# ipl-uw/ZeDO-Release

Hardware: AMD Instinct MI355X
Metric: poses/sec (1000-step sampler, H=50) (higher is better)
Workload: dtype f32; 1 GPU; BASELINE configs[2] (3DPW pw3d_test, H=50, 1000 steps): N=1015 poses/GPU x H=50 hypotheses, IPO 500 it (17 joints) + 1000 OIL steps + P1/P2 min-over-hypotheses selection; random-init ScoreModelFC_Adv weights, synthetic detections; settings=pw3d, rows_per_gpu=50750, poses_total=1015

## Files before the change

### include/zedo_hip.h

```cpp
#ifndef ZEDO_HIP_H
#define ZEDO_HIP_H

#include <stddef.h>
#include <stdint.h>

#ifdef __cplusplus
extern "C" {
#endif

#define ZEDO_ABI_VERSION 5

#define ZEDO_OK 0
#define ZEDO_E_BADARG (-1)
#define ZEDO_E_NOGPU (-2)
#define ZEDO_E_WORKSPACE (-3)

typedef struct zedo_weights zedo_weights_t;
typedef struct zedo_schedule zedo_schedule_t;

int zedo_abi_version(void);
const char *zedo_error_string(int code);

int zedo_weights_create(const float *h_params, size_t n_floats, int n_joints, int joint_dim, int hidden,
                        int embed, int n_blocks, void *stream, zedo_weights_t **out);
void zedo_weights_destroy(zedo_weights_t *w);

#define ZEDO_MATH_F32 0
#define ZEDO_MATH_F16X3 1
int zedo_weights_set_math(zedo_weights_t *w, int mode, void *stream);
int zedo_weights_get_math(const zedo_weights_t *w);

int zedo_schedule_create(const zedo_weights_t *w, const float *h_t, int S, float label_scale, float beta_min,
                         float beta_max, int n_sde, void *stream, zedo_schedule_t **out);
void zedo_schedule_destroy(zedo_schedule_t *s);
int zedo_schedule_read(const zedo_schedule_t *s, float *h_tbias, float *h_a, float *h_c);

size_t zedo_workspace_bytes(int B);

int zedo_reproj_prepare(const float *d_uv, const float *d_K, const float *d_conf, int N, int J,
                        float *d_geom, float *d_conf_clamped, void *stream);

int zedo_reproj_degenerate(const float *d_geom, int N, int J, int *h_count, void *stream);

// ... 47 lines not shown
```

### zedo-release_amd/csrc/zedo_capi.hip

```cpp
#include "../../include/zedo_hip.h"
#include "zedo_internal.h"

#include <algorithm>
#include <atomic>
#include <cmath>
#include <cstdlib>
#include <cstring>
#include <mutex>
#include <new>
#include <vector>

using namespace zedo;

struct zedo_weights {
    int J3, hidden, embed, n_blocks;
    float *d_all;
    const float *W_pre;
    const float *W_hid[4];
    const float *W_post;
    const float *b_post;
    const float *gamma[NLAYER], *beta[NLAYER];
    const float *W_s, *b_s;
    const float *W_t[NLAYER];
    const float *b_sum[NLAYER];
    float *d_scratch;
    std::mutex scratch_mu;
    int math;
    uint16_t *d_W16;
    float wmax_hid[6];
    float act_bound;
    float unscale[6];
    bool finite16;
    float row_ratio16;
};

struct zedo_schedule {
    int S, Sp, nl, hidden;
    float *d_tbias;
    std::vector<float> a, c;
};

#define HIPCHK(x)                      \
    do {                               \
        hipError_t e_ = (x);           \
        if (e_ != hipSuccess) return (int)e_; \
    } while (0)

static inline int round_up(int v, int m) { return (v + m - 1) / m * m; }
static int check_device();
static int check_device_fwd() { return check_device(); }

namespace {
struct Prof {
// ... 134 lines not shown
        case ZEDO_E_NOGPU: return "zedo: no gfx950 device";
        case ZEDO_E_WORKSPACE: return "zedo: workspace too small";
    }
    return code > 0 ? hipGetErrorString((hipError_t)code) : "zedo: unknown error";
}

static int check_device() {
    int dev = 0;
    if (hipGetDevice(&dev) != hipSuccess) return ZEDO_E_NOGPU;
    hipDeviceProp_t p;
    if (hipGetDeviceProperties(&p, dev) != hipSuccess) return ZEDO_E_NOGPU;
    if (strncmp(p.gcnArchName, "gfx950", 6) != 0) return ZEDO_E_NOGPU;
    return ZEDO_OK;
}

extern "C" int zedo_weights_create(const float *h_params, size_t n_floats, int n_joints, int joint_dim, int hidden,
                                   int embed, int n_blocks, void *stream, zedo_weights_t **out) {
    if (!h_params || !out) return ZEDO_E_BADARG;
    const int J3 = n_joints * joint_dim;
    if (hidden != HID || embed != EMB || n_blocks != 2 || J3 < 1 || J3 > XLD) return ZEDO_E_BADARG;
    const size_t H = hidden, E = embed;
    const size_t expect = (H * J3 + H) + (H * E + H) + 2 * H + (E * E + E) + 4 * ((H * H + H) + (H * E + H) + 2 * H) +
                          ((size_t)J3 * H + J3);
    if (n_floats != expect) return ZEDO_E_BADARG;
    if (int rc = check_device()) return rc;
    hipStream_t st = (hipStream_t)stream;

    size_t off = 0;
    auto take = [&](size_t n) { size_t o = off; off += (n + 63) / 64 * 64; return o; };
    const size_t o_Wpre = take(H * XLD), o_Whid0 = take(4 * H * H), o_Wpost = take((size_t)XLD * H), o_bpost = take(XLD);
    const size_t o_gamma = take(NLAYER * H), o_beta = take(NLAYER * H), o_Ws = take(E * E), o_bs = take(E);
    const size_t o_Wt = take(NLAYER * H * E), o_bsum = take(NLAYER * H);
    std::vector<float> img(off, 0.0f);

    const float *p = h_params;
    auto next = [&](size_t n) { const float *q = p; p += n; return q; };
    float wmax_hid_tmp[6] = {0, 0, 0, 0, 0, 0};
    float gn_bound[NLAYER] = {0, 0, 0, 0, 0};
    bool finite = true;
    auto all_finite = [&](const float *v, size_t n) {
        for (size_t q = 0; q < n; ++q) finite &= (bool)std::isfinite(v[q]);
    };
    float row_ratio = 1.0f;
    auto row_ratio_of = [&](const float *wm, size_t rows, size_t cols, float mat_max) {
        if (!(mat_max > 0.f)) return;
        for (size_t r = 0; r < rows; ++r) {
            float rm = 0.f;
// ... 29 lines not shown
        for (size_t q = 0; q < H * H; ++q) wm = std::fmax(wm, std::fabs(w[q]));
        all_finite(w, H * H);
        wmax_hid_tmp[l - 1] = wm;
        row_ratio_of(w, H, H, wm);
        memcpy(&img[o_Wt + (size_t)l * H * E], wt, sizeof(float) * H * E);
        memcpy(&img[o_gamma + (size_t)l * H], g, sizeof(float) * H);
        memcpy(&img[o_beta + (size_t)l * H], be, sizeof(float) * H);
        for (size_t n = 0; n < H; ++n) img[o_bsum + (size_t)l * H + n] = bt[n] + b[n];
    }
    const float *w_post = next((size_t)J3 * H), *b_post = next(J3);
    memcpy(&img[o_Wpost], w_post, sizeof(float) * J3 * H);
    for (size_t q = 0; q < (size_t)J3 * H; ++q) wmax_hid_tmp[5] = std::fmax(wmax_hid_tmp[5], std::fabs(w_post[q]));
    all_finite(w_post, (size_t)J3 * H);
    row_ratio_of(w_post, J3, H, wmax_hid_tmp[5]);
    memcpy(&img[o_bpost], b_post, sizeof(float) * J3);

    zedo_weights *w = new (std::nothrow) zedo_weights();
    if (!w) return (int)hipErrorOutOfMemory;
    w->J3 = J3; w->hidden = hidden; w->embed = embed; w->n_blocks = n_blocks;
    w->d_scratch = nullptr;
    w->math = ZEDO_MATH_F32; w->d_W16 = nullptr;
    for (int l = 0; l < 6; ++l) { w->wmax_hid[l] = wmax_hid_tmp[l]; w->unscale[l] = 1.0f; }
    w->act_bound = std::fmax(std::fmax(gn_bound[1], gn_bound[3]), gn_bound[0] + gn_bound[2] + gn_bound[4]);
    w->finite16 = finite;
    w->row_ratio16 = row_ratio;
    hipError_t e = hipMalloc(&w->d_all, off * sizeof(float));
    if (e == hipSuccess) e = hipMalloc(&w->d_scratch, sizeof(float) * ((size_t)2 * ROW_PAD * EMB + ROW_PAD));
    if (e != hipSuccess) { (void)hipFree(w->d_all); delete w; return (int)e; }
    e = hipMemcpyAsync(w->d_all, img.data(), off * sizeof(float), hipMemcpyHostToDevice, st);
    if (e == hipSuccess) e = hipStreamSynchronize(st);
    if (e != hipSuccess) { (void)hipFree(w->d_all); (void)hipFree(w->d_scratch); delete w; return (int)e; }
    const float *d = w->d_all;
    w->W_pre = d + o_Wpre;
    for (int l = 0; l < 4; ++l) w->W_hid[l] = d + o_Whid0 + (size_t)l * H * H;
    w->W_post = d + o_Wpost; w->b_post = d + o_bpost;
    for (int l = 0; l < NLAYER; ++l) {
        w->gamma[l] = d + o_gamma + (size_t)l * H; w->beta[l] = d + o_beta + (size_t)l * H;
        w->W_t[l] = d + o_Wt + (size_t)l * H * E;  w->b_sum[l] = d + o_bsum + (size_t)l * H;
    }
    w->W_s = d + o_Ws; w->b_s = d + o_bs;
    *out = w;
    return ZEDO_OK;
}

extern "C" void zedo_weights_destroy(zedo_weights_t *w) {
    if (!w) return;
    (void)hipFree(w->d_all);
    (void)hipFree(w->d_scratch);
    (void)hipFree(w->d_W16);
    delete w;
}

extern "C" int zedo_weights_get_math(const zedo_weights_t *w) { return w ? w->math : ZEDO_E_BADARG; }

extern "C" int zedo_weights_set_math(zedo_weights_t *w, int mode, void *stream) {
// ... 37 lines not shown
    s->a.resize(S); s->c.resize(S);
    for (int i = 0; i < S; ++i) {
        const double t = (double)h_t[i] * ((double)label_scale / 999.0), b0 = (double)beta_min, b1 = (double)beta_max;
        const double beta = b0 + t * (b1 - b0);
        const double disc = 1.0 - std::exp(-2.0 * b0 * t - (b1 - b0) * t * t);
        const double sd = 1.0 - std::exp(2.0 * (-0.25 * t * t * (b1 - b0) - 0.5 * t * b0));
        s->a[i] = (float)(1.0 + 0.5 * beta / n_sde);
        s->c[i] = (float)(-(beta * disc) / (n_sde * sd));
#ifdef ZEDO_MUT_SDE_C
        s->c[i] = (float)(-(beta * disc) / (n_sde * sd) * (1.0 + 1e-4));
#endif
    }
    const bool borrow = Sp == ROW_PAD;
    std::unique_lock<std::mutex> lk(const_cast<zedo_weights_t *>(w)->scratch_mu, std::defer_lock);
    float *d_t = nullptr, *d_pe = nullptr, *d_temb = nullptr;
    s->d_tbias = nullptr;
    hipError_t e = hipSuccess;
    if (borrow) {
        lk.lock();
        d_pe = w->d_scratch; d_temb = d_pe + (size_t)ROW_PAD * EMB; d_t = d_temb + (size_t)ROW_PAD * EMB;
    } else {
        e = hipMalloc(&d_t, sizeof(float) * S);
        if (e == hipSuccess) e = hipMalloc(&d_pe, sizeof(float) * (size_t)Sp * EMB);
        if (e == hipSuccess) e = hipMalloc(&d_temb, sizeof(float) * (size_t)Sp * EMB);
    }
    if (e == hipSuccess) e = hipMalloc(&s->d_tbias, sizeof(float) * (size_t)Sp * NLAYER * HID);
    if (e == hipSuccess) e = hipMemcpyAsync(d_t, h_t, sizeof(float) * S, hipMemcpyHostToDevice, st);
    if (e == hipSuccess) e = launch_posemb(d_t, S, Sp, label_scale, d_pe, st);
    if (e == hipSuccess) {
        LayerArgs a{};
        a.X = d_pe; a.ldx = EMB; a.W = w->W_s; a.ldw = EMB; a.bias = w->b_s; a.out = d_temb; a.ldo = EMB;
        a.K = EMB; a.N = EMB; a.Mp = Sp;
        e = launch_layer(a, EPI_BIAS_SILU, st);
    }
    for (int l = 0; l < NLAYER && e == hipSuccess; ++l) {
        LayerArgs a{};
        a.X = d_temb; a.ldx = EMB; a.W = w->W_t[l]; a.ldw = EMB; a.bias = w->b_sum[l];
        a.out = s->d_tbias + (size_t)l * HID; a.ldo = NLAYER * HID; a.K = EMB; a.N = HID; a.Mp = Sp;
        e = launch_layer(a, EPI_BIAS, st);
    }
    {
        const hipError_t es = hipStreamSynchronize(st);
        if (e == hipSuccess) e = es;
    }
    if (!borrow) { (void)hipFree(d_t); (void)hipFree(d_pe); (void)hipFree(d_temb); }
    if (e != hipSuccess) { (void)hipFree(s->d_tbias); delete s; return (int)e; }
    *out = s;
    return ZEDO_OK;
}

extern "C" void zedo_schedule_destroy(zedo_schedule_t *s) {
    if (!s) return;
    (void)hipFree(s->d_tbias);
    delete s;
}

extern "C" int zedo_schedule_read(const zedo_schedule_t *s, float *h_tbias, float *h_a, float *h_c) {
    if (!s) return ZEDO_E_BADARG;
    if (h_tbias) HIPCHK(hipMemcpy(h_tbias, s->d_tbias, sizeof(float) * (size_t)s->S * NLAYER * HID, hipMemcpyDeviceToHost));
    if (h_a) memcpy(h_a, s->a.data(), sizeof(float) * s->S);
    if (h_c) memcpy(h_c, s->c.data(), sizeof(float) * s->S);
    return ZEDO_OK;
}

static inline size_t ws_rows(int B) { return (size_t)round_up((int)std::min((size_t)B, chunk_rows_cap()), BATCH_PAD); }

extern "C" size_t zedo_workspace_bytes(int B) {
    if (B < 1) return 0;
// ... 33 lines not shown
    int solve = 0, B = 0, N = 0;
    long long row0 = 0;
};

struct Net {
    const zedo_weights *w;
    float *xpad, *h, *h1;
    int Bp, ld;
    hipStream_t st;
    bool f16() const { return w->math == ZEDO_MATH_F16X3; }
    const uint16_t *W_pre16() const { return w->d_W16 + 4 * (size_t)HID * HID * 2; }
    const uint16_t *W_post16() const { return W_pre16() + (size_t)HID * XLD * 2; }

    LayerArgs pre_args(const float *tb) const {
        LayerArgs a{};
        a.Mp = Bp; a.X = xpad; a.ldx = XLD; a.W = w->W_pre; a.ldw = XLD; a.K = XLD; a.N = HID;
        a.kzero8 = w->J3 <= XLD - 8;
        a.bias = tb; a.gamma = w->gamma[0]; a.beta = w->beta[0]; a.out = h; a.ldo = HID;
        return a;
    }
    Layer16Args pre_args16(const float *tb) const {
        Layer16Args b{};
        b.K = XLD; b.N = HID; b.Mp = Bp; b.ldo = ld; b.Xf32 = xpad; b.W = W_pre16(); b.unscale = w->unscale[4];
        b.bias = tb; b.gamma = w->gamma[0]; b.beta = w->beta[0]; b.out = h; b.out_f32 = 0;
        return b;
    }
    LayerArgs post_args(bool sde, float sa, float sc, float *eps_out, const NextReproj &nr) const {
        LayerArgs a{};
        a.Mp = Bp; a.X = h; a.ldx = HID; a.W = w->W_post; a.ldw = HID; a.K = HID; a.N = XLD; a.bias = w->b_post; a.ldo = XLD;
        a.scratch = h1 + (size_t)Bp * XLD;
        if (sde) {
            a.out = xpad; a.sde_a = sa; a.sde_c = sc;
            a.rp_geom = nr.geom; a.rp_T = nr.T; a.rp_solve = nr.solve; a.rp_B = nr.B; a.rp_N = nr.N; a.rp_row0 = nr.row0;
// ... 26 lines not shown
            const int l1 = 1 + 2 * blk, l2 = 2 + 2 * blk;
            if (f16()) {
                const size_t per = (size_t)HID * HID * 2;
                Layer16Args b{};
                b.K = HID; b.N = HID; b.Mp = Bp; b.ldx = b.ldo = ld; b.out_f32 = 0;
                b.X = reinterpret_cast<const uint16_t *>(h); b.W = w->d_W16 + (size_t)(l1 - 1) * per; b.unscale = w->unscale[l1 - 1];
                b.bias = tb + (size_t)l1 * HID; b.gamma = w->gamma[l1]; b.beta = w->beta[l1]; b.out = h1;
                { ProfScope ps(ZEDO_PROF_HIDDEN, st); b.clk = ps.clk; e = launch_layer16(b, EPI_GN_SILU, st); b.clk = nullptr; }
                if (e != hipSuccess) break;
                b.X = reinterpret_cast<const uint16_t *>(h1); b.W = w->d_W16 + (size_t)(l2 - 1) * per; b.unscale = w->unscale[l2 - 1];
                b.bias = tb + (size_t)l2 * HID; b.gamma = w->gamma[l2]; b.beta = w->beta[l2];
                b.res = reinterpret_cast<const uint16_t *>(h); b.out = h;
                { ProfScope ps(ZEDO_PROF_HIDDEN, st); b.clk = ps.clk; e = launch_layer16(b, EPI_GN_SILU_RES, st); b.clk = nullptr; }
            } else {
                LayerArgs a{};
                a.Mp = Bp; a.X = h; a.ldx = HID; a.W = w->W_hid[l1 - 1]; a.ldw = HID; a.K = HID; a.N = HID;
                a.bias = tb + (size_t)l1 * HID; a.gamma = w->gamma[l1]; a.beta = w->beta[l1]; a.out = h1; a.ldo = HID;
                { ProfScope ps(ZEDO_PROF_HIDDEN, st); a.clk = ps.clk; e = launch_layer(a, EPI_GN_SILU, st); a.clk = nullptr; }
                if (e != hipSuccess) break;
                a.X = h1; a.W = w->W_hid[l2 - 1];
                a.bias = tb + (size_t)l2 * HID; a.gamma = w->gamma[l2]; a.beta = w->beta[l2]; a.out = h;
                { ProfScope ps(ZEDO_PROF_HIDDEN, st); a.clk = ps.clk; e = launch_layer(a, EPI_GN_SILU_RES, st); a.clk = nullptr; }
            }
        }
        return e;
    }
    hipError_t post(bool sde, float sa, float sc, float *eps_out, const NextReproj &nr) const {
        ProfScope ps(ZEDO_PROF_POST, st);
        if (f16()) return launch_layer16(post_args16(sde, sa, sc, eps_out, nr), sde ? EPI_SDE : EPI_BIAS, st);
        return launch_layer(post_args(sde, sa, sc, eps_out, nr), sde ? EPI_SDE : EPI_BIAS, st);
    }
    hipError_t all(const float *tb, bool sde, float sa, float sc, float *eps_out, const NextReproj &nr = NextReproj()) const {
        hipError_t e = pre(tb);
        if (e == hipSuccess) e = hidden(tb);
        if (e == hipSuccess) e = post(sde, sa, sc, eps_out, nr);
        return e;
    }
};

struct Ws { float *xpad, *h, *h1; size_t rows; };
static Ws carve(void *ws, int B) {
    Ws r; r.rows = ws_rows(B);
    r.xpad = (float *)ws; r.h = r.xpad + r.rows * XLD; r.h1 = r.h + r.rows * HID;
    return r;
}

static int step_common(const zedo_weights_t *w, const zedo_schedule_t *s, int step, const float *d_x_in, float *d_out,
                       bool sde, int B, void *ws, size_t ws_bytes, hipStream_t st) {
    if (!w || !s || !d_x_in || !d_out || !ws || B < 1 || step < 0 || step >= s->S) return ZEDO_E_BADARG;
    if (ws_bytes < zedo_workspace_bytes(B)) return ZEDO_E_WORKSPACE;
    const size_t cap = chunk_rows_cap();
    const float *tb = s->d_tbias + (size_t)step * NLAYER * HID;
    for (size_t r0 = 0; r0 < (size_t)B; r0 += cap) {
        const int Bc = (int)std::min(cap, (size_t)B - r0), Bp = round_up(Bc, BATCH_PAD);
        Ws k = carve(ws, B);
        HIPCHK(launch_pack_rows(d_x_in + r0 * w->J3, k.xpad, Bc, Bp, w->J3, st));
        const Net net{w, k.xpad, k.h, k.h1, Bp, (int)k.rows, st};
        if (sde) {
            HIPCHK(net.all(tb, true, s->a[step], s->c[step], nullptr));
            HIPCHK(launch_unpack_rows(k.xpad, d_out + r0 * w->J3, Bc, w->J3, st));
        } else {
            HIPCHK(net.all(tb, false, 0.f, 0.f, k.h1));
            HIPCHK(launch_unpack_rows(k.h1, d_out + r0 * w->J3, Bc, w->J3, st));
        }
    }
    return ZEDO_OK;
}
// ... 24 lines not shown
        Ws k = carve(d_workspace, B);
        HIPCHK(launch_pack_rows(d_x + r0 * w->J3, k.xpad, Bc, Bp, w->J3, st));
        static const bool unfused = getenv("ZEDO_UNFUSED_REPROJ") != nullptr;
        const Net net{w, k.xpad, k.h, k.h1, Bp, (int)k.rows, st};
        for (int i = step_begin; i < step_end; ++i) {
            if (i == step_begin || unfused) {
                ProfScope ps(ZEDO_PROF_REPROJ, st);
                HIPCHK(launch_reproj_step_padded(k.xpad, d_geom, d_T + r0 * 3, i >= switch_step, Bc, N,
                                                 row_offset + (long long)r0, st));
            }
            NextReproj nr;
            if (i + 1 < step_end && !unfused) {
                nr.geom = d_geom; nr.T = d_T + r0 * 3; nr.solve = (i + 1) >= switch_step; nr.B = Bc; nr.N = N;
                nr.row0 = row_offset + (long long)r0;
            }
            HIPCHK(net.all(s->d_tbias + (size_t)i * NLAYER * HID, true, s->a[i], s->c[i], nullptr, nr));
        }
        HIPCHK(launch_unpack_rows(k.xpad, d_x + r0 * w->J3, Bc, w->J3, st));
    }
    return ZEDO_OK;
}

extern "C" int zedo_ipo_fit_resume(const float *d_x0, const float *d_uv, const float *d_K, const int *h_keylist, int k,
                                   int axes_mask, float ipo_T, float min_scale, float max_scale, int iters,
                                   double normaliser, float *d_R, float *d_T, float *d_q, float *d_scale,
                                   float *d_state, int it_begin, int B, int H, int N, int J, long long row_offset,
                                   void *stream) {
    if (!d_x0 || !d_uv || !d_K || !h_keylist || !d_R || !d_T || B < 1 || H < 1 || N < 1 || J < 1 || k < 1 || k > 17 ||
        iters < 0 || it_begin < 0 || (it_begin > 0 && !d_state) || !(normaliser > 0) || row_offset < 0)
        return ZEDO_E_BADARG;
    if (row_offset + (long long)B > (long long)H * N) return ZEDO_E_BADARG;
// ... 38 lines not shown
```

### zedo-release_amd/csrc/zedo_gemm.hip

```cpp
#include "zedo_internal.h"
#include "zedo_tile.h"

#include <atomic>
#include <cstdlib>

#ifdef ZEDO_UBENCH
#include "../../tools/ubench/zedo_tile_hooks.inc"
#else
#define TL_MARK(var)
#define TL_FLUSH(t0, t1, t2)
#endif

namespace zedo {

template <int BM, int BN, int WM, int WN, int EPI, int NBUF = 2, int BK = 32, int SCHED = 0, int KSKIP = 0, int KQ = 1>
__device__ __forceinline__ void layer_tile(const LayerArgs &a, const int m0, const int n0, const int out_m0) {
    constexpr int NW = WM * WN;
    constexpr int CPR = BK / 4;
    constexpr int RPD = 64 / CPR;
    constexpr int KG = BK / 8;
    static_assert(BK == 32 || BK == 16, "BK");
    constexpr int TM = BM / WM, TN = BN / WN;
    constexpr int TJ = TM / 32, TI = TN / 32;
    constexpr int IA = BN / RPD / NW, IB = BM / RPD / NW;
// ... 27 lines not shown
        else
            dma16(Xbase + (size_t)kt * (BK * 4) + (size_t)(p - IA) * (RPD * 4) * a.ldx, xlane,
                  lds0 + (unsigned)(((NBUF * BN + buf * BM + (wid * IB + (p - IA)) * RPD) * BK) * 4));
    };
    auto dma = [&](int kt, int buf) {
#pragma unroll
        for (int p = 0; p < IPW; ++p) dma_one(kt, buf, p);
    };

    const int fswz = (BK == 32) ? (li & 7) : ((li >> 2) & 3);
    int foff[KG];
#pragma unroll
    for (int kg = 0; kg < KG; ++kg) foff[kg] = ((2 * kg + kh) ^ fswz) * 4;
    const float *Ab0 = As + (wn * TN + li) * BK;
    const float *Bb0 = Bs + (wm * TM + li) * BK;
    f32x4 fa0[TI], fb0[TJ], fa1[TI], fb1[TJ];
    auto fread = [&](f32x4(&fa)[TI], f32x4(&fb)[TJ], int buf, int kg) {
#pragma unroll
        for (int i = 0; i < TI; ++i) fa[i] = *reinterpret_cast<const f32x4 *>(Ab0 + (buf * BN + i * 32) * BK + foff[kg]);
#pragma unroll
        for (int j = 0; j < TJ; ++j) fb[j] = *reinterpret_cast<const f32x4 *>(Bb0 + (buf * BM + j * 32) * BK + foff[kg]);
    };
    f32x16 acc[TI][TJ];
#pragma unroll
    for (int i = 0; i < TI; ++i)
#pragma unroll
        for (int j = 0; j < TJ; ++j)
#pragma unroll
            for (int e = 0; e < 16; ++e) acc[i][j][e] = 0.0f;
    auto mma = [&](const f32x4(&fa)[TI], const f32x4(&fb)[TJ]) {
#pragma unroll
        for (int e = 0; e < 4; ++e)
#pragma unroll
            for (int i = 0; i < TI; ++i)
#pragma unroll
                for (int j = 0; j < TJ; ++j)
                    acc[i][j] = __builtin_amdgcn_mfma_f32_32x32x2f32(fa[i][e], fb[j][e], acc[i][j], 0, 0, 0);
    };
    constexpr int H1 = (IPW + 1) / 2, H2 = IPW - H1;
    auto mma_dma = [&](const f32x4(&fa)[TI], const f32x4(&fb)[TJ], int kt, int buf, int p0, int cnt) {
#pragma unroll
        for (int e = 0; e < 4; ++e) {
#pragma unroll
            for (int q = 0; q < 4; ++q)
                if (q < cnt && q * 4 / cnt == e) {
                    dma_one(kt, buf, p0 + q);
                    __builtin_amdgcn_sched_barrier(0);
// ... 12 lines not shown
    TL_MARK(tl0)
    if (EPI != EPI_PARTIAL && tid < BN / 4) {
        *reinterpret_cast<f32x4 *>(Ps + tid * 4) = *reinterpret_cast<const f32x4 *>(a.bias + n0 + tid * 4);
        if constexpr (EPI == EPI_GN_SILU || EPI == EPI_GN_SILU_RES) {
            *reinterpret_cast<f32x4 *>(Ps + BN + tid * 4) = *reinterpret_cast<const f32x4 *>(a.gamma + n0 + tid * 4);
            *reinterpret_cast<f32x4 *>(Ps + 2 * BN + tid * 4) = *reinterpret_cast<const f32x4 *>(a.beta + n0 + tid * 4);
        }
    }
    const int KT = a.K / BK;
    f32x16 qsum[KQ > 1 ? TI : 1][KQ > 1 ? TJ : 1];
    const int KTQ = KT / KQ;
#pragma unroll
    for (int t = 0; t < NBUF; ++t) dma(min(t, KT - 1), t);
    asm volatile("s_waitcnt vmcnt(%0)" ::"n"((NBUF - 1) * IPW) : "memory");
    __syncthreads();
    fread(fa0, fb0, 0, 0);
    TL_MARK(tl1)
    for (int kt0 = 0; kt0 < KT; kt0 += NBUF) {
#pragma unroll
      for (int buf = 0; buf < NBUF; ++buf) {
        const int kt = kt0 + buf;
        const int nxt = (buf + 1 == NBUF) ? 0 : buf + 1;
        const int prv = (buf == 0) ? NBUF - 1 : buf - 1;
        fread(fa1, fb1, buf, 1);
        if constexpr (SCHED & 1) __builtin_amdgcn_sched_barrier(0);
        if constexpr (SCHED & 2) mma_dma(fa0, fb0, min(kt - 1 + NBUF, KT - 1), prv, H1, H2);
        else mma(fa0, fb0);
        if constexpr (KG == 4) {
            fread(fa0, fb0, buf, 2);
            if constexpr (SCHED & 1) __builtin_amdgcn_sched_barrier(0);
            mma(fa1, fb1);
            if constexpr (SCHED & 1) __builtin_amdgcn_sched_barrier(0);
            fread(fa1, fb1, buf, 3);
            if constexpr (SCHED & 1) __builtin_amdgcn_sched_barrier(0);
            mma(fa0, fb0);
        }
        const bool skip_last = KSKIP == 1 && KG == 4 && buf == NBUF - 1;
        asm volatile("s_waitcnt vmcnt(%0)" ::"n"((NBUF - 2) * IPW) : "memory");
        __syncthreads();
        if (skip_last) {
        } else if constexpr (SCHED & 2) {
            fread(fa0, fb0, nxt, 0);
            __builtin_amdgcn_sched_barrier(0);
            mma_dma(fa1, fb1, min(kt + NBUF, KT - 1), buf, 0, H1);
        } else {
            dma(min(kt + NBUF, KT - 1), buf);
            fread(fa0, fb0, nxt, 0);
            if constexpr (SCHED & 1) __builtin_amdgcn_sched_barrier(0);
            mma(fa1, fb1);
            if constexpr (SCHED & 1) __builtin_amdgcn_sched_barrier(0);
        }
      }
// ... 44 lines not shown
                    __builtin_amdgcn_global_load_lds(
                        (const __attribute__((address_space(1))) void *)(reinterpret_cast<const char *>(obase) +
                                                                         ((unsigned)grow * (unsigned)a.ldo + (unsigned)((pos ^ (sr & 7)) * 4)) * 4u),
                        (__attribute__((address_space(3))) void *)(S + idx * RPI * BN), 16, 0, 0);
                }
                asm volatile("s_waitcnt vmcnt(0)" ::: "memory");
                __syncthreads();
            }
#pragma unroll
            for (int i = 0; i < TI; ++i) {
                float o[16];
                f32x4 b4[4], ga[4], be[4];
                const float *pc = Ps + wn * TN + i * 32 + 4 * kh;
#pragma unroll
                for (int g = 0; g < 4; ++g) {
                    b4[g] = *reinterpret_cast<const f32x4 *>(pc + 8 * g);
                    if constexpr (EPI == EPI_GN_SILU || EPI == EPI_GN_SILU_RES) {
                        ga[g] = *reinterpret_cast<const f32x4 *>(pc + BN + 8 * g);
                        be[g] = *reinterpret_cast<const f32x4 *>(pc + 2 * BN + 8 * g);
                    }
                }
                epilogue_values<EPI>(acc[i][j], b4, ga, be, a.sde_c, o);
                float *srow = S + (wm * 32 + li) * BN;
#pragma unroll
                for (int g = 0; g < 4; ++g) {
                    const int c = (wn * TN + i * 32 + 8 * g + 4 * kh) >> 2;
                    f32x4 *slot = reinterpret_cast<f32x4 *>(srow + ((c ^ (li & 7)) << 2));
                    f32x4 v = {o[4 * g], o[4 * g + 1], o[4 * g + 2], o[4 * g + 3]};
                    if constexpr (EPI == EPI_GN_SILU_RES) {
                        const f32x4 h = *slot;
#pragma unroll
                        for (int e = 0; e < 4; ++e) v[e] += h[e];
                    } else if constexpr (EPI == EPI_SDE) {
                        const f32x4 x = *slot;
#pragma unroll
                        for (int e = 0; e < 4; ++e) v[e] = __builtin_fmaf(a.sde_a, x[e], v[e]);
                    }
// ... 133 lines not shown
        if (a.Mp % bm) return 1e30;
        const long tiles = (long)(a.Mp / bm) * ncol;
        const long rounds = (tiles + (long)cus * slots_per_cu - 1) / ((long)cus * slots_per_cu);
        return rounds * 6.0 + (double)((tiles + cus - 1) / cus) * tile_us;
    };
    const double kdepth = a.K / 1024.0;
    const double c32 = cost(32, 3, 14.5 * kdepth), c64 = cost(64, 3, 28.2 * kdepth), c128 = cost(128, 2, 55.1 * kdepth);
    if (c32 <= c64 && c32 <= c128) return launch_cfg<32, 128, 1, 4, EPI, 2, 32, SCHED_THIN>(a, st);
    if (c64 <= c128) return launch_cfg<64, 128, 2, 4, EPI, 2, 32, SCHED_THIN>(a, st);
    return launch_cfg<128, 128, 2, 2, EPI, 2, 32, SCHED_BIG, PLAIN_WPE>(a, st);
}

template <int EPI>
static hipError_t launch_wide(const LayerArgs &a, hipStream_t st) {
    if (a.K <= 64) {
        if (a.K == 64 && a.kzero8) return launch_cfg<64, 128, 2, 4, EPI, 2, 32, SCHED_THIN, 1, 1>(a, st);
        return launch_cfg<64, 128, 2, 4, EPI, 2, 32, SCHED_THIN>(a, st);
    }
    constexpr int WG_PER_CU = 3;
    constexpr int W8 = (EPI == EPI_GN_SILU_RES) ? 1 : 0;
    const int per_round = num_cus() * WG_PER_CU * 128 / (a.N / 128);
    int rows_big = (a.Mp / per_round) * per_round;
    if (rows_big == 0) {
        const int one_each = num_cus() * 128 / (a.N / 128);
        const int mix_big = (a.Mp / one_each) * one_each;
        constexpr int SMR = (W8 ? 64 : 32);
        if (mix_big > 0 && a.Mp > mix_big && (a.Mp - mix_big) % SMR == 0) {
            const double kd = a.K / 1024.0;
            const long small_tiles = (long)((a.Mp - mix_big) / SMR) * (a.N / 128);
            const double est_mix = (mix_big / one_each) * 55.1 * kd + (double)((small_tiles + num_cus() - 1) / num_cus()) * (W8 ? 28.2 : 13.9) * kd + 6.0;
            auto single = [&](int bm, int slots, double t) {
// ... 137 lines not shown
```

### zedo-release_amd/csrc/zedo_internal.h

```cpp
#pragma once
#include <hip/hip_runtime.h>
#include <stddef.h>
#include <stdint.h>

#include <atomic>

namespace zedo {

constexpr int MAX_DEVICES = 16;
inline int device_slot() {
    int dev = 0;
    if (hipGetDevice(&dev) != hipSuccess) return -1;
    return (dev >= 0 && dev < MAX_DEVICES) ? dev : -1;
}
inline hipError_t allow_lds(const void *kern, size_t lds, std::atomic<bool> *done ) {
    const int slot = device_slot();
    if (slot < 0 || !done[slot].load(std::memory_order_acquire)) {
        hipError_t e = hipFuncSetAttribute(kern, hipFuncAttributeMaxDynamicSharedMemorySize, (int)lds);
        if (e != hipSuccess) return e;
        if (slot >= 0) done[slot].store(true, std::memory_order_release);
    }
    return hipSuccess;
}
inline int num_cus() {
// ... 26 lines not shown
    EPI_PARTIAL = 5,
};

struct LayerArgs {
    const float *X;
    const float *W;
    const float *bias;
    const float *gamma;
    const float *beta;
    float *out;
    int ldx, ldw, ldo;
    int K;
    int N;
    int Mp;
    float sde_a, sde_c;
    int kzero8;
    long long *clk;
    const float *rp_geom;
    float *rp_T;
    int rp_solve, rp_B, rp_N;
    long long rp_row0;
    float *scratch;
};
constexpr int POST_SPLIT_ROWS = 2048;

hipError_t launch_layer(const LayerArgs &a, int epilogue, hipStream_t st);

struct Layer16Args {
    const uint16_t *X;
    int ldx, ldo;
    const uint16_t *W;
// ... 88 lines not shown
```

### zedo-release_amd/csrc/zedo_tile.h

```cpp
#pragma once
#include "zedo_internal.h"

namespace zedo {

typedef float f32x16 __attribute__((ext_vector_type(16)));
typedef float f32x2 __attribute__((ext_vector_type(2)));
typedef _Float16 f16x8 __attribute__((ext_vector_type(8)));
typedef _Float16 f16x4 __attribute__((ext_vector_type(4)));

__device__ __forceinline__ void split_f16x8(const f32x4 &v0, const f32x4 &v1, f16x8 &h, f16x8 &l) {
#pragma unroll
    for (int e = 0; e < 4; ++e) {
        const _Float16 h0 = (_Float16)v0[e], h1 = (_Float16)v1[e];
        h[e] = h0; h[4 + e] = h1;
        l[e] = (_Float16)(v0[e] - (float)h0); l[4 + e] = (_Float16)(v1[e] - (float)h1);
    }
}
__device__ __forceinline__ float join_f16(_Float16 h, _Float16 l) { return (float)h + (float)l; }


__device__ __forceinline__ void dma16(const char *sbase, unsigned voff, unsigned lds_byte_addr) {
    unsigned keep;
    asm volatile("s_mov_b32 %0, m0\n\ts_mov_b32 m0, %3\n\ts_nop 0\n\tglobal_load_lds_dwordx4 %2, %1\n\ts_mov_b32 m0, %0"
                 : "=&s"(keep)
// ... 3 lines not shown

template <int N>
__device__ __forceinline__ void dma16n(const char *sbase, unsigned voff, unsigned lds_byte_addr) {
    static_assert(N == 1 || N == 2 || N == 4, "pieces per M0 write (offsets up to 3072 fit the 13-bit signed field)");
    unsigned keep;
    if constexpr (N == 4)
        asm volatile("s_mov_b32 %0, m0\n\ts_mov_b32 m0, %3\n\ts_nop 0\n\tglobal_load_lds_dwordx4 %2, %1\n\tglobal_load_lds_dwordx4 %2, %1 offset:1024\n\t"
                     "global_load_lds_dwordx4 %2, %1 offset:2048\n\tglobal_load_lds_dwordx4 %2, %1 offset:3072\n\ts_mov_b32 m0, %0"
                     : "=&s"(keep) : "s"(sbase), "v"(voff), "s"(lds_byte_addr) : "memory");
    else if constexpr (N == 2)
        asm volatile("s_mov_b32 %0, m0\n\ts_mov_b32 m0, %3\n\ts_nop 0\n\tglobal_load_lds_dwordx4 %2, %1\n\tglobal_load_lds_dwordx4 %2, %1 offset:1024\n\ts_mov_b32 m0, %0"
                     : "=&s"(keep) : "s"(sbase), "v"(voff), "s"(lds_byte_addr) : "memory");
    else
        asm volatile("s_mov_b32 %0, m0\n\ts_mov_b32 m0, %3\n\ts_nop 0\n\tglobal_load_lds_dwordx4 %2, %1\n\ts_mov_b32 m0, %0"
                     : "=&s"(keep) : "s"(sbase), "v"(voff), "s"(lds_byte_addr) : "memory");
}

__device__ __forceinline__ float silu_fast(float y) {
    return y * __builtin_amdgcn_rcpf(1.0f + __builtin_amdgcn_exp2f(y * -1.44269504088896340736f));
}

template <int EPI, bool SCALED = false, bool PACKED = true>
__device__ __forceinline__ void epilogue_values(const f32x16 &acc, const f32x4 (&b4)[4], const f32x4 (&ga)[4],
                                                const f32x4 (&be)[4], float sde_c, float (&o)[16], float acc_scale = 1.0f) {
    if constexpr ((EPI == EPI_GN_SILU || EPI == EPI_GN_SILU_RES) && !PACKED) {
        float p[16];
#pragma unroll
        for (int k = 0; k < 16; ++k) {
            const float b = b4[k >> 2][k & 3];
            if constexpr (SCALED) p[k] = __builtin_fmaf(acc[k], acc_scale, b);
// ... 97 lines not shown
```

### zedo-release_amd/zedo_hip/__init__.py

```python
import ctypes
import os

import numpy as np
import torch

_HERE = os.path.dirname(os.path.abspath(__file__))


def _load_zedo_build():
    import importlib.util
    import sys
    if "zedo_build" in sys.modules:
        return sys.modules["zedo_build"]
    spec = importlib.util.spec_from_file_location("zedo_build", os.path.join(os.path.dirname(_HERE), "zedo_build.py"))
    mod = importlib.util.module_from_spec(spec)
    sys.modules["zedo_build"] = mod
    spec.loader.exec_module(mod)
    return mod


_zb = _load_zedo_build()

LIB_PATH = _zb.ensure_library()

_lib = ctypes.CDLL(LIB_PATH)

_vp, _i, _f, _d, _ll, _sz = (ctypes.c_void_p, ctypes.c_int, ctypes.c_float, ctypes.c_double,
                             ctypes.c_longlong, ctypes.c_size_t)

SIGNATURES = {
    "zedo_abi_version": (_i, []),
    "zedo_error_string": (ctypes.c_char_p, [_i]),
    "zedo_weights_create": (_i, [_vp, _sz, _i, _i, _i, _i, _i, _vp, ctypes.POINTER(_vp)]),
    "zedo_weights_destroy": (None, [_vp]),
    "zedo_weights_set_math": (_i, [_vp, _i, _vp]),
    "zedo_weights_get_math": (_i, [_vp]),
    "zedo_schedule_create": (_i, [_vp, _vp, _i, _f, _f, _f, _i, _vp, ctypes.POINTER(_vp)]),
    "zedo_schedule_destroy": (None, [_vp]),
    "zedo_schedule_read": (_i, [_vp, _vp, _vp, _vp]),
    "zedo_workspace_bytes": (_sz, [_i]),
    "zedo_reproj_prepare": (_i, [_vp, _vp, _vp, _i, _i, _vp, _vp, _vp]),
    "zedo_reproj_degenerate": (_i, [_vp, _i, _i, _vp, _vp]),
    "zedo_reproj_grad": (_i, [_vp, _vp, _vp, _i, _vp, _i, _i, _i, _ll, _vp]),
    "zedo_score_eps": (_i, [_vp, _vp, _i, _vp, _vp, _i, _vp, _sz, _vp]),
    "zedo_sde_step": (_i, [_vp, _vp, _i, _vp, _i, _vp, _sz, _vp]),
    "zedo_oil_run": (_i, [_vp, _vp, _vp, _vp, _vp, _i, _i, _i, _i, _i, _ll, _vp, _sz, _vp]),
    "zedo_ipo_fit": (_i, [_vp, _vp, _vp, _vp, _i, _i, _f, _f, _f, _i, _d, _vp, _vp, _vp, _vp, _i, _i, _i, _i, _ll, _vp]),
    "zedo_ipo_fit_resume": (_i, [_vp, _vp, _vp, _vp, _i, _i, _f, _f, _f, _i, _d, _vp, _vp, _vp, _vp, _vp, _i, _i, _i, _i,
                                 _i, _ll, _vp]),
    "zedo_rotate_init": (_i, [_vp, _vp, _vp, _i, _i, _i, _i, _ll, _vp]),
    "zedo_min_mpjpe": (_i, [_vp, _vp, _i, _i, _i, _ll, _i, _vp, _vp, _vp, _vp]),
# ... 342 lines not shown
```

Baseline: 319.3 poses/s.

## Fold GroupNorm mean-centring into pre-centred weights and biases for f32 path

Precomputes, at weight load, copies of the pre, hidden and time-embedding weights and biases with the GroupNorm per-group (32-channel) mean subtracted. The GEMM output is then already centred, so the epilogue only needs a variance reduction. The biases are loaded into the accumulators at init instead of being added afterwards. The gamma and beta are pre-scaled by -log2(e) so the SiLU exp2 needs fewer ops. It also adds a K-skip variant that drops more zero-padded K slices in the first layer. This costs extra weight and tbias memory, and changes the rounding of the f32 path.

Measured after the change: 320.9 poses/s, median of 6. About the same (+0.5%).

```diff
diff --git a/include/zedo_hip.h b/include/zedo_hip.h
--- a/include/zedo_hip.h
+++ b/include/zedo_hip.h
@@ -27,6 +27,7 @@
 
 #define ZEDO_MATH_F32 0
 #define ZEDO_MATH_F16X3 1
+int zedo_gn_centre(const float *h_in, int rows, int cols, float *h_out);
 int zedo_weights_set_math(zedo_weights_t *w, int mode, void *stream);
 int zedo_weights_get_math(const zedo_weights_t *w);
 
diff --git a/zedo-release_amd/csrc/zedo_capi.hip b/zedo-release_amd/csrc/zedo_capi.hip
--- a/zedo-release_amd/csrc/zedo_capi.hip
+++ b/zedo-release_amd/csrc/zedo_capi.hip
@@ -23,6 +23,8 @@
     const float *W_s, *b_s;
     const float *W_t[NLAYER];
     const float *b_sum[NLAYER];
+    const float *W_pre_c, *W_hid_c[4], *W_t_c[NLAYER], *b_sum_c[NLAYER];
+    const float *gamma_f[NLAYER], *beta_f[NLAYER];
     float *d_scratch;
     std::mutex scratch_mu;
     int math;
@@ -37,6 +39,7 @@
 struct zedo_schedule {
     int S, Sp, nl, hidden;
     float *d_tbias;
+    float *d_tbias_c;
     std::vector<float> a, c;
 };
 
@@ -201,6 +204,23 @@
     return ZEDO_OK;
 }
 
+static void gn_centre(const float *in, size_t rows, size_t cols, float *out) {
+    std::vector<double> m(cols);
+    for (size_t g = 0; g < rows; g += 32) {
+        std::fill(m.begin(), m.end(), 0.0);
+        for (size_t r = g; r < g + 32; ++r)
+            for (size_t c = 0; c < cols; ++c) m[c] += (double)in[r * cols + c];
+        for (size_t r = g; r < g + 32; ++r)
+            for (size_t c = 0; c < cols; ++c) out[r * cols + c] = (float)((double)in[r * cols + c] - m[c] * (1.0 / 32.0));
+    }
+}
+
+extern "C" int zedo_gn_centre(const float *h_in, int rows, int cols, float *h_out) {
+    if (!h_in || !h_out || rows < 32 || rows % 32 || cols < 1) return ZEDO_E_BADARG;
+    gn_centre(h_in, (size_t)rows, (size_t)cols, h_out);
+    return ZEDO_OK;
+}
+
 extern "C" int zedo_weights_create(const float *h_params, size_t n_floats, int n_joints, int joint_dim, int hidden,
                                    int embed, int n_blocks, void *stream, zedo_weights_t **out) {
     if (!h_params || !out) return ZEDO_E_BADARG;
@@ -218,6 +238,8 @@
     const size_t o_Wpre = take(H * XLD), o_Whid0 = take(4 * H * H), o_Wpost = take((size_t)XLD * H), o_bpost = take(XLD);
     const size_t o_gamma = take(NLAYER * H), o_beta = take(NLAYER * H), o_Ws = take(E * E), o_bs = take(E);
     const size_t o_Wt = take(NLAYER * H * E), o_bsum = take(NLAYER * H);
+    const size_t o_Wpre_c = take(H * XLD), o_Whid_c = take(4 * H * H), o_Wt_c = take(NLAYER * H * E), o_bsum_c = take(NLAYER * H);
+    const size_t o_gamma_f = take(NLAYER * H), o_beta_f = take(NLAYER * H);
     std::vector<float> img(off, 0.0f);
 
     const float *p = h_params;
@@ -277,6 +299,14 @@
     all_finite(w_post, (size_t)J3 * H);
     row_ratio_of(w_post, J3, H, wmax_hid_tmp[5]);
     memcpy(&img[o_bpost], b_post, sizeof(float) * J3);
+    gn_centre(&img[o_Wpre], H, XLD, &img[o_Wpre_c]);
+    gn_centre(&img[o_Whid0], 4 * H, H, &img[o_Whid_c]);
+    gn_centre(&img[o_Wt], NLAYER * H, E, &img[o_Wt_c]);
+    gn_centre(&img[o_bsum], NLAYER * H, 1, &img[o_bsum_c]);
+    for (size_t q = 0; q < NLAYER * H; ++q) {
+        img[o_gamma_f + q] = (float)(-1.4426950408889634074 * (double)img[o_gamma + q]);
+        img[o_beta_f + q] = (float)(-1.4426950408889634074 * (double)img[o_beta + q]);
+    }
 
     zedo_weights *w = new (std::nothrow) zedo_weights();
     if (!w) return (int)hipErrorOutOfMemory;
@@ -302,6 +332,12 @@
         w->W_t[l] = d + o_Wt + (size_t)l * H * E;  w->b_sum[l] = d + o_bsum + (size_t)l * H;
     }
     w->W_s = d + o_Ws; w->b_s = d + o_bs;
+    w->W_pre_c = d + o_Wpre_c;
+    for (int l = 0; l < 4; ++l) w->W_hid_c[l] = d + o_Whid_c + (size_t)l * H * H;
+    for (int l = 0; l < NLAYER; ++l) {
+        w->W_t_c[l] = d + o_Wt_c + (size_t)l * H * E;  w->b_sum_c[l] = d + o_bsum_c + (size_t)l * H;
+        w->gamma_f[l] = d + o_gamma_f + (size_t)l * H; w->beta_f[l] = d + o_beta_f + (size_t)l * H;
+    }
     *out = w;
     return ZEDO_OK;
 }
@@ -369,7 +405,7 @@
     const bool borrow = Sp == ROW_PAD;
     std::unique_lock<std::mutex> lk(const_cast<zedo_weights_t *>(w)->scratch_mu, std::defer_lock);
     float *d_t = nullptr, *d_pe = nullptr, *d_temb = nullptr;
-    s->d_tbias = nullptr;
+    s->d_tbias = s->d_tbias_c = nullptr;
     hipError_t e = hipSuccess;
     if (borrow) {
         lk.lock();
@@ -380,6 +416,7 @@
         if (e == hipSuccess) e = hipMalloc(&d_temb, sizeof(float) * (size_t)Sp * EMB);
     }
     if (e == hipSuccess) e = hipMalloc(&s->d_tbias, sizeof(float) * (size_t)Sp * NLAYER * HID);
+    if (e == hipSuccess) e = hipMalloc(&s->d_tbias_c, sizeof(float) * (size_t)Sp * NLAYER * HID);
     if (e == hipSuccess) e = hipMemcpyAsync(d_t, h_t, sizeof(float) * S, hipMemcpyHostToDevice, st);
     if (e == hipSuccess) e = launch_posemb(d_t, S, Sp, label_scale, d_pe, st);
     if (e == hipSuccess) {
@@ -388,10 +425,12 @@
         a.K = EMB; a.N = EMB; a.Mp = Sp;
         e = launch_layer(a, EPI_BIAS_SILU, st);
     }
-    for (int l = 0; l < NLAYER && e == hipSuccess; ++l) {
+    for (int l = 0; l < 2 * NLAYER && e == hipSuccess; ++l) {
+        const bool c = l >= NLAYER;
+        const int k = l % NLAYER;
         LayerArgs a{};
-        a.X = d_temb; a.ldx = EMB; a.W = w->W_t[l]; a.ldw = EMB; a.bias = w->b_sum[l];
-        a.out = s->d_tbias + (size_t)l * HID; a.ldo = NLAYER * HID; a.K = EMB; a.N = HID; a.Mp = Sp;
+        a.X = d_temb; a.ldx = EMB; a.W = c ? w->W_t_c[k] : w->W_t[k]; a.ldw = EMB; a.bias = c ? w->b_sum_c[k] : w->b_sum[k];
+        a.out = (c ? s->d_tbias_c : s->d_tbias) + (size_t)k * HID; a.ldo = NLAYER * HID; a.K = EMB; a.N = HID; a.Mp = Sp;
         e = launch_layer(a, EPI_BIAS, st);
     }
     {
@@ -399,7 +438,7 @@
         if (e == hipSuccess) e = es;
     }
     if (!borrow) { (void)hipFree(d_t); (void)hipFree(d_pe); (void)hipFree(d_temb); }
-    if (e != hipSuccess) { (void)hipFree(s->d_tbias); delete s; return (int)e; }
+    if (e != hipSuccess) { (void)hipFree(s->d_tbias); (void)hipFree(s->d_tbias_c); delete s; return (int)e; }
     *out = s;
     return ZEDO_OK;
 }
@@ -407,6 +446,7 @@
 extern "C" void zedo_schedule_destroy(zedo_schedule_t *s) {
     if (!s) return;
     (void)hipFree(s->d_tbias);
+    (void)hipFree(s->d_tbias_c);
     delete s;
 }
 
@@ -470,9 +510,9 @@
 
     LayerArgs pre_args(const float *tb) const {
         LayerArgs a{};
-        a.Mp = Bp; a.X = xpad; a.ldx = XLD; a.W = w->W_pre; a.ldw = XLD; a.K = XLD; a.N = HID;
-        a.kzero8 = w->J3 <= XLD - 8;
-        a.bias = tb; a.gamma = w->gamma[0]; a.beta = w->beta[0]; a.out = h; a.ldo = HID;
+        a.Mp = Bp; a.X = xpad; a.ldx = XLD; a.W = w->W_pre_c; a.ldw = XLD; a.K = XLD; a.N = HID;
+        a.kzero = XLD - w->J3;
+        a.bias = tb; a.gamma = w->gamma_f[0]; a.beta = w->beta_f[0]; a.out = h; a.ldo = HID;
         return a;
     }
     Layer16Args pre_args16(const float *tb) const {
@@ -529,12 +569,12 @@
                 { ProfScope ps(ZEDO_PROF_HIDDEN, st); b.clk = ps.clk; e = launch_layer16(b, EPI_GN_SILU_RES, st); b.clk = nullptr; }
             } else {
                 LayerArgs a{};
-                a.Mp = Bp; a.X = h; a.ldx = HID; a.W = w->W_hid[l1 - 1]; a.ldw = HID; a.K = HID; a.N = HID;
-                a.bias = tb + (size_t)l1 * HID; a.gamma = w->gamma[l1]; a.beta = w->beta[l1]; a.out = h1; a.ldo = HID;
+                a.Mp = Bp; a.X = h; a.ldx = HID; a.W = w->W_hid_c[l1 - 1]; a.ldw = HID; a.K = HID; a.N = HID;
+                a.bias = tb + (size_t)l1 * HID; a.gamma = w->gamma_f[l1]; a.beta = w->beta_f[l1]; a.out = h1; a.ldo = HID;
                 { ProfScope ps(ZEDO_PROF_HIDDEN, st); a.clk = ps.clk; e = launch_layer(a, EPI_GN_SILU, st); a.clk = nullptr; }
                 if (e != hipSuccess) break;
-                a.X = h1; a.W = w->W_hid[l2 - 1];
-                a.bias = tb + (size_t)l2 * HID; a.gamma = w->gamma[l2]; a.beta = w->beta[l2]; a.out = h;
+                a.X = h1; a.W = w->W_hid_c[l2 - 1];
+                a.bias = tb + (size_t)l2 * HID; a.gamma = w->gamma_f[l2]; a.beta = w->beta_f[l2]; a.out = h;
                 { ProfScope ps(ZEDO_PROF_HIDDEN, st); a.clk = ps.clk; e = launch_layer(a, EPI_GN_SILU_RES, st); a.clk = nullptr; }
             }
         }
@@ -553,6 +593,10 @@
     }
 };
 
+static const float *tbias_rows(const zedo_weights *w, const zedo_schedule *s, int step) {
+    return (w->math == ZEDO_MATH_F16X3 ? s->d_tbias : s->d_tbias_c) + (size_t)step * NLAYER * HID;
+}
+
 struct Ws { float *xpad, *h, *h1; size_t rows; };
 static Ws carve(void *ws, int B) {
     Ws r; r.rows = ws_rows(B);
@@ -565,7 +609,7 @@
     if (!w || !s || !d_x_in || !d_out || !ws || B < 1 || step < 0 || step >= s->S) return ZEDO_E_BADARG;
     if (ws_bytes < zedo_workspace_bytes(B)) return ZEDO_E_WORKSPACE;
     const size_t cap = chunk_rows_cap();
-    const float *tb = s->d_tbias + (size_t)step * NLAYER * HID;
+    const float *tb = tbias_rows(w, s, step);
     for (size_t r0 = 0; r0 < (size_t)B; r0 += cap) {
         const int Bc = (int)std::min(cap, (size_t)B - r0), Bp = round_up(Bc, BATCH_PAD);
         Ws k = carve(ws, B);
@@ -620,7 +664,7 @@
                 nr.geom = d_geom; nr.T = d_T + r0 * 3; nr.solve = (i + 1) >= switch_step; nr.B = Bc; nr.N = N;
                 nr.row0 = row_offset + (long long)r0;
             }
-            HIPCHK(net.all(s->d_tbias + (size_t)i * NLAYER * HID, true, s->a[i], s->c[i], nullptr, nr));
+            HIPCHK(net.all(tbias_rows(w, s, i), true, s->a[i], s->c[i], nullptr, nr));
         }
         HIPCHK(launch_unpack_rows(k.xpad, d_x + r0 * w->J3, Bc, w->J3, st));
     }
diff --git a/zedo-release_amd/csrc/zedo_gemm.hip b/zedo-release_amd/csrc/zedo_gemm.hip
--- a/zedo-release_amd/csrc/zedo_gemm.hip
+++ b/zedo-release_amd/csrc/zedo_gemm.hip
@@ -65,6 +65,7 @@
     for (int kg = 0; kg < KG; ++kg) foff[kg] = ((2 * kg + kh) ^ fswz) * 4;
     const float *Ab0 = As + (wn * TN + li) * BK;
     const float *Bb0 = Bs + (wm * TM + li) * BK;
+    constexpr bool GN = (EPI == EPI_GN_SILU || EPI == EPI_GN_SILU_RES);
     f32x4 fa0[TI], fb0[TJ], fa1[TI], fb1[TJ];
     auto fread = [&](f32x4(&fa)[TI], f32x4(&fb)[TJ], int buf, int kg) {
 #pragma unroll
@@ -73,15 +74,17 @@
         for (int j = 0; j < TJ; ++j) fb[j] = *reinterpret_cast<const f32x4 *>(Bb0 + (buf * BM + j * 32) * BK + foff[kg]);
     };
     f32x16 acc[TI][TJ];
-#pragma unroll
-    for (int i = 0; i < TI; ++i)
-#pragma unroll
-        for (int j = 0; j < TJ; ++j)
-#pragma unroll
-            for (int e = 0; e < 16; ++e) acc[i][j][e] = 0.0f;
-    auto mma = [&](const f32x4(&fa)[TI], const f32x4(&fb)[TJ]) {
-#pragma unroll
-        for (int e = 0; e < 4; ++e)
+    if constexpr (!GN) {
+#pragma unroll
+        for (int i = 0; i < TI; ++i)
+#pragma unroll
+            for (int j = 0; j < TJ; ++j)
+#pragma unroll
+                for (int e = 0; e < 16; ++e) acc[i][j][e] = 0.0f;
+    }
+    auto mma = [&](const f32x4(&fa)[TI], const f32x4(&fb)[TJ], int ne = 4) {
+#pragma unroll
+        for (int e = 0; e < ne; ++e)
 #pragma unroll
             for (int i = 0; i < TI; ++i)
 #pragma unroll
@@ -124,6 +127,21 @@
     for (int t = 0; t < NBUF; ++t) dma(min(t, KT - 1), t);
     asm volatile("s_waitcnt vmcnt(%0)" ::"n"((NBUF - 1) * IPW) : "memory");
     __syncthreads();
+    if constexpr (GN) {
+#pragma unroll
+        for (int j = 0; j < TJ; ++j)
+#pragma unroll
+            for (int i = 0; i < TI; ++i) {
+                const float *pc = Ps + wn * TN + i * 32 + 4 * kh;
+#pragma unroll
+                for (int g = 0; g < 4; ++g) {
+                    const f32x4 b = *reinterpret_cast<const f32x4 *>(pc + 8 * g);
+#pragma unroll
+                    for (int e = 0; e < 4; ++e) acc[i][j][4 * g + e] = b[e];
+                }
+                asm volatile("" ::: "memory");
+            }
+    }
     fread(fa0, fb0, 0, 0);
     TL_MARK(tl1)
     for (int kt0 = 0; kt0 < KT; kt0 += NBUF) {
@@ -143,9 +161,9 @@
             if constexpr (SCHED & 1) __builtin_amdgcn_sched_barrier(0);
             fread(fa1, fb1, buf, 3);
             if constexpr (SCHED & 1) __builtin_amdgcn_sched_barrier(0);
-            mma(fa0, fb0);
-        }
-        const bool skip_last = KSKIP == 1 && KG == 4 && buf == NBUF - 1;
+            mma(fa0, fb0, (KSKIP == 2 && buf == NBUF - 1) ? 3 : 4);
+        }
+        const bool skip_last = KSKIP >= 1 && KG == 4 && buf == NBUF - 1;
         asm volatile("s_waitcnt vmcnt(%0)" ::"n"((NBUF - 2) * IPW) : "memory");
         __syncthreads();
         if (skip_last) {
@@ -220,13 +238,15 @@
                 const float *pc = Ps + wn * TN + i * 32 + 4 * kh;
 #pragma unroll
                 for (int g = 0; g < 4; ++g) {
-                    b4[g] = *reinterpret_cast<const f32x4 *>(pc + 8 * g);
-                    if constexpr (EPI == EPI_GN_SILU || EPI == EPI_GN_SILU_RES) {
+                    if constexpr (GN) {
                         ga[g] = *reinterpret_cast<const f32x4 *>(pc + BN + 8 * g);
                         be[g] = *reinterpret_cast<const f32x4 *>(pc + 2 * BN + 8 * g);
+                    } else {
+                        b4[g] = *reinterpret_cast<const f32x4 *>(pc + 8 * g);
                     }
                 }
-                epilogue_values<EPI>(acc[i][j], b4, ga, be, a.sde_c, o);
+                if constexpr (GN) gn_silu_centred(acc[i][j], ga, be, o);
+                else epilogue_values<EPI>(acc[i][j], b4, ga, be, a.sde_c, o);
                 float *srow = S + (wm * 32 + li) * BN;
 #pragma unroll
                 for (int g = 0; g < 4; ++g) {
@@ -390,7 +410,8 @@
 template <int EPI>
 static hipError_t launch_wide(const LayerArgs &a, hipStream_t st) {
     if (a.K <= 64) {
-        if (a.K == 64 && a.kzero8) return launch_cfg<64, 128, 2, 4, EPI, 2, 32, SCHED_THIN, 1, 1>(a, st);
+        if (a.K == 64 && a.kzero >= 13) return launch_cfg<64, 128, 2, 4, EPI, 2, 32, SCHED_THIN, 1, 2>(a, st);
+        if (a.K == 64 && a.kzero >= 8) return launch_cfg<64, 128, 2, 4, EPI, 2, 32, SCHED_THIN, 1, 1>(a, st);
         return launch_cfg<64, 128, 2, 4, EPI, 2, 32, SCHED_THIN>(a, st);
     }
     constexpr int WG_PER_CU = 3;
diff --git a/zedo-release_amd/csrc/zedo_internal.h b/zedo-release_amd/csrc/zedo_internal.h
--- a/zedo-release_amd/csrc/zedo_internal.h
+++ b/zedo-release_amd/csrc/zedo_internal.h
@@ -64,7 +64,7 @@
     int N;
     int Mp;
     float sde_a, sde_c;
-    int kzero8;
+    int kzero;
     long long *clk;
     const float *rp_geom;
     float *rp_T;
diff --git a/zedo-release_amd/csrc/zedo_tile.h b/zedo-release_amd/csrc/zedo_tile.h
--- a/zedo-release_amd/csrc/zedo_tile.h
+++ b/zedo-release_amd/csrc/zedo_tile.h
@@ -41,6 +41,37 @@
     else
         asm volatile("s_mov_b32 %0, m0\n\ts_mov_b32 m0, %3\n\ts_nop 0\n\tglobal_load_lds_dwordx4 %2, %1\n\ts_mov_b32 m0, %0"
                      : "=&s"(keep) : "s"(sbase), "v"(voff), "s"(lds_byte_addr) : "memory");
+}
+
+__device__ __forceinline__ void gn_silu_centred(const f32x16 &p, const f32x4 (&ga)[4], const f32x4 (&be)[4], float (&o)[16]) {
+    f32x2 q2 = {0.0f, 0.0f};
+#pragma unroll
+    for (int k = 0; k < 8; ++k) {
+        const f32x2 p2 = {p[2 * k], p[2 * k + 1]};
+        q2 = __builtin_elementwise_fma(p2, p2, q2);
+    }
+    float qs = q2.x + q2.y;
+    qs += __shfl_xor(qs, 32);
+#ifdef ZEDO_MUT_GN_EPS
+    constexpr float GN_EPS = 2e-5f;
+#else
+    constexpr float GN_EPS = 1e-5f;
+#endif
+    const float rstd = __builtin_amdgcn_rsqf(__builtin_fmaf(qs, 1.0f / 32.0f, GN_EPS));
+    constexpr float K = -1.44269504088896340736f;
+    const f32x2 r2 = {rstd, rstd}, k2 = {K, K};
+#pragma unroll
+    for (int k = 0; k < 8; ++k) {
+        const f32x2 p2 = {p[2 * k], p[2 * k + 1]};
+        const f32x2 g2 = {ga[k >> 1][2 * (k & 1)], ga[k >> 1][2 * (k & 1) + 1]};
+        const f32x2 e2 = {be[k >> 1][2 * (k & 1)], be[k >> 1][2 * (k & 1) + 1]};
+        const f32x2 t = __builtin_elementwise_fma(p2, r2 * g2, e2);
+        const f32x2 x = {__builtin_amdgcn_exp2f(t.x), __builtin_amdgcn_exp2f(t.y)};
+        const f32x2 d = __builtin_elementwise_fma(x, k2, k2);
+        const f32x2 v = t * (f32x2){__builtin_amdgcn_rcpf(d.x), __builtin_amdgcn_rcpf(d.y)};
+        o[2 * k] = v.x;
+        o[2 * k + 1] = v.y;
+    }
 }
 
 __device__ __forceinline__ float silu_fast(float y) {
diff --git a/zedo-release_amd/zedo_hip/__init__.py b/zedo-release_amd/zedo_hip/__init__.py
--- a/zedo-release_amd/zedo_hip/__init__.py
+++ b/zedo-release_amd/zedo_hip/__init__.py
@@ -35,6 +35,7 @@
     "zedo_weights_destroy": (None, [_vp]),
     "zedo_weights_set_math": (_i, [_vp, _i, _vp]),
     "zedo_weights_get_math": (_i, [_vp]),
+    "zedo_gn_centre": (_i, [_vp, _i, _i, _vp]),
     "zedo_schedule_create": (_i, [_vp, _vp, _i, _f, _f, _f, _i, _vp, ctypes.POINTER(_vp)]),
     "zedo_schedule_destroy": (None, [_vp]),
     "zedo_schedule_read": (_i, [_vp, _vp, _vp, _vp]),
```
